# eloialonso/diamond

Hardware: AMD Instinct MI355X
Metric: imagined frames/sec (64x64, 3 denoise steps, batch 256) (higher is better)
Workload: dtype f32 via split-f16 MFMA (world-model convs (3x3 stride 1 / 2, 1x1): fp32 operands split into 2 x fp16 pieces, 3 x v_mfma_f32_*_f16 per product, fp32 accumulate (fp32-class, 22-bit operands); attention core, linears: exact fp32 v_mfma_f32_16x16x4_f32; actor-critic encoder forward, dgrad and weight-gra

## Files before the change

diamond_amd/csrc/dmd_conv.hip:

```cpp
#include <stdlib.h>

#include "dmd_common.h"

#define DMD_CIN_MAX 256

template <int WN_, bool CFGB_, int TAPS_, int STRIDE_, bool SPLIT_ = false>
struct ConvGeom {
  static constexpr bool SPLIT = SPLIT_;
  static constexpr int WN = WN_;
  static constexpr int WM = 4 / WN_;
  static constexpr int MB = 8 / WM;
  static constexpr bool CFGB = CFGB_;
  static constexpr int SUB = CFGB_ ? 2 : 1;
  static constexpr int TH = 8;
  static constexpr int TW = CFGB_ ? 8 : 16;
  static constexpr int TAPS = TAPS_;
  static constexpr int S = STRIDE_;
  static constexpr int PAD = TAPS_ == 9 ? 1 : 0;
  static constexpr int PH = (TH - 1) * STRIDE_ + 1 + 2 * PAD;
  static constexpr int PW = (TW - 1) * STRIDE_ + 1 + 2 * PAD;
  static constexpr int NPP = SUB * PH * PW;
  static constexpr int ITEMS = (NPP * 4 + 255) / 256;
  static constexpr int NBUF = STRIDE_ == 2 ? 1 : 2;
  static constexpr int MIN_WAVES = (WN_ == 4 && CFGB_ && TAPS_ == 9 && STRIDE_ == 1) ? 1 : 2;
  static constexpr bool GENG = false;
};

template <int WN_, bool CFGB_, int TAPS_, int STRIDE_, bool SPLIT_ = false>
struct ConvGeomGN : ConvGeom<WN_, CFGB_, TAPS_, STRIDE_, SPLIT_> {
  static constexpr bool GENG = true;
};

template <class G>
__device__ __forceinline__ void conv_norm_entry(const dmd_norm& nm, int n, int c, int C, int hv, int wv, float* m, float* a, float* ad) {
  if (G::GENG) {
    const int gs = dmd_gn_group_size(C);
    norm_entry_gs(nm, n, c, C, gs, (double)gs * hv * wv, m, a, ad);
  } else {
    norm_entry(nm, n, c, C, (double)DMD_GN_GROUP * hv * wv, m, a, ad);
  }
}

typedef _Float16 h4 __attribute__((ext_vector_type(4)));

__device__ __forceinline__ f32x4 split_h4l4(f32x4 v) {
  h4 hh, ll;
#pragma unroll
  for (int e = 0; e < 4; ++e) {
    hh[e] = (_Float16)v[e];
    ll[e] = (_Float16)(v[e] - (float)hh[e]);
  }
  const uint2 a = __builtin_bit_cast(uint2, hh), b = __builtin_bit_cast(uint2, ll);
  return __builtin_bit_cast(f32x4, (uint4){a.x, a.y, b.x, b.y});
}

struct TileInfo {
  int n, y0, x0;
  bool valid;
};

template <class G>
__device__ __forceinline__ TileInfo decode_subtile(const dmd_conv_params& p, int tile, int s) {
  const int tiles_x = p.W / G::TW, tiles_y = p.H / G::TH;
  const int per_img = tiles_x * tiles_y;
  const int gs = tile * G::SUB + s;
  TileInfo t;
  t.valid = gs < p.N * per_img;
  const int g2 = t.valid ? gs : 0;
  t.n = g2 / per_img;
  const int r = g2 - t.n * per_img;
  const int ty = r / tiles_x;
  t.y0 = ty * G::TH;
  t.x0 = (r - ty * tiles_x) * G::TW;
  return t;
}

template <int SUB>
__device__ __forceinline__ TileInfo pick_tile(const TileInfo* ti, int s) {
  return (SUB == 2 && s) ? ti[SUB - 1] : ti[0];
}

template <class G>
__global__ __launch_bounds__(256, G::MIN_WAVES) void conv_mfma_kernel(const dmd_conv_params p) {
  __shared__ f32x4 patch[G::NBUF][G::NPP * 4];
  __shared__ float tab_mean[G::SUB][DMD_CIN_MAX];
  __shared__ float tab_a[G::SUB][DMD_CIN_MAX];
  __shared__ float tab_add[G::SUB][DMD_CIN_MAX];
  __shared__ float rtab[G::SUB][3][64];
  __shared__ double red[G::SUB][4][2];

  const int tid = threadIdx.x;
  const int lane = tid & 63;
  const int wave = tid >> 6;
  const int wn = wave % G::WN;
  const int wm = wave / G::WN;
  const int j = lane & 15;
  const int kg = lane >> 4;
  const int tile = blockIdx.x;
  const int cout_group0 = blockIdx.y * (16 * G::WN);

  TileInfo ti[G::SUB];
#pragma unroll
  for (int s = 0; s < G::SUB; ++s) ti[s] = decode_subtile<G>(p, tile, s);

  const int up = p.upsample;
  const int Hin = p.H * G::S, Win = p.W * G::S;
  const int Hs = Hin >> up, Ws = Win >> up;
  const int Hvo = p.valid_h ? p.valid_h : p.H, Wvo = p.valid_w ? p.valid_w : p.W;
  const int Hvi = Hvo * G::S, Wvi = Wvo * G::S;
  const int Hvs = Hvi >> up, Wvs = Wvi >> up;
  const int C0 = p.src[0].C;
  const int C1 = p.nsrc > 1 ? p.src[1].C : 0;
  const int nch0 = C0 >> 4;
  const int nchunks = (C0 + C1) >> 4;

  for (int c = tid; c < C0 + C1; c += 256) {
    const int si = c < C0 ? 0 : 1;
    const dmd_conv_src& sc = p.src[si];
    const int cl = si ? c - C0 : c;
#pragma unroll
    for (int s = 0; s < G::SUB; ++s) {
      float m = 0.f, a = 1.f, ad = 0.f;
      if (sc.prologue != DMD_PROLOGUE_NONE && ti[s].valid)
        conv_norm_entry<G>(sc.norm, ti[s].n, cl, sc.C, Hvs, Wvs, &m, &a, &ad);
      tab_mean[s][c] = m;
      tab_a[s][c] = a;
      tab_add[s][c] = ad;
    }
  }
  if (p.residual_norm.stats) {
    for (int c = tid; c < 16 * G::WN; c += 256) {
#pragma unroll
      for (int s = 0; s < G::SUB; ++s) {
        float m = 0.f, a = 1.f, ad = 0.f;
        const int cc = cout_group0 + c;
        if (ti[s].valid && cc < p.Cout)
          conv_norm_entry<G>(p.residual_norm, ti[s].n, cc, p.Cout, Hvo, Wvo, &m, &a, &ad);
        rtab[s][0][c] = m;
        rtab[s][1][c] = a;
        rtab[s][2][c] = ad;
      }
    }
  }

  int goff[G::ITEMS];
  int loff[G::ITEMS];
  int isub[G::ITEMS];
  const int q = tid & 3;
#pragma unroll
  for (int it = 0; it < G::ITEMS; ++it) {
    const int id = it * 256 + tid;
    const int pp = id >> 2;
    const bool ok = pp < G::NPP;
    const int s = G::SUB == 1 ? 0 : (pp >= G::PH * G::PW ? 1 : 0);
    const TileInfo t = pick_tile<G::SUB>(ti, s);
    const int rem = pp - s * (G::PH * G::PW);
    const int py = rem / G::PW;
    const int px = rem - py * G::PW;
    const int iy = t.y0 * G::S - G::PAD + py;
    const int ix = t.x0 * G::S - G::PAD + px;
    const bool inb = ok && t.valid && iy >= 0 && iy < Hvi && ix >= 0 && ix < Wvi;
    goff[it] = inb ? ((t.n * Hs + (iy >> up)) * Ws + (ix >> up)) : -1;
    loff[it] = ok ? pp * 4 + ((q + 2 * (pp >> 2)) & 3) : -1;
    isub[it] = s;
  }

  int pixbase[G::MB];
#pragma unroll
  for (int mb = 0; mb < G::MB; ++mb) {
    const int gmb = wm * G::MB + mb;
    int s, y, x;
    if (G::CFGB) {
      s = gmb >> 2;
      y = (gmb & 3) * 2 + (j >> 3);
      x = j & 7;
    } else {
      s = 0;
      y = gmb;
      x = j;
    }
    pixbase[mb] = s * (G::PH * G::PW) + (y * G::S) * G::PW + x * G::S;
  }

  f32x4 acc[G::MB];
#pragma unroll
  for (int mb = 0; mb < G::MB; ++mb) acc[mb] = (f32x4){0.f, 0.f, 0.f, 0.f};

  const size_t wstep = (size_t)p.CoutPad * 16;
  const float* wlane = p.w + (size_t)(cout_group0 + 16 * wn + j) * 16 + 4 * kg;

  f32x4 stage[G::ITEMS];
  auto load_chunk = [&](int ck) {
    const int si = ck < nch0 ? 0 : 1;
    const dmd_conv_src& sc = p.src[si];
    const int c0 = (si ? ck - nch0 : ck) * 16 + 4 * q;
#pragma unroll
    for (int it = 0; it < G::ITEMS; ++it) {
      stage[it] = (f32x4){0.f, 0.f, 0.f, 0.f};
      if (goff[it] >= 0) stage[it] = *(const f32x4*)(sc.x + (size_t)goff[it] * sc.C + c0);
    }
  };
  const bool fast_math = p.precision != DMD_PRECISION_F32;
  auto store_chunk = [&](int ck, int buf) {
    const int si = ck < nch0 ? 0 : 1;
    const int prologue = p.src[si].prologue;
    const int cc = ck * 16 + 4 * q;
#pragma unroll
    for (int it = 0; it < G::ITEMS; ++it) {
      f32x4 v = stage[it];
      if (prologue != DMD_PROLOGUE_NONE && goff[it] >= 0) {
        const int s = isub[it];
#pragma unroll
        for (int e = 0; e < 4; ++e) {
          float t = (v[e] - tab_mean[s][cc + e]) * tab_a[s][cc + e] + tab_add[s][cc + e];
          if (prologue == DMD_PROLOGUE_NORM_SILU) t = fast_math ? dmd_silu_fast(t) : dmd_silu(t);
          v[e] = t;
        }
      }
      if (G::SPLIT) v = split_h4l4(v);
      if (loff[it] >= 0) patch[buf][loff[it]] = v;
    }
  };

  f32x4 wreg[G::TAPS];
  auto load_weights = [&](int ck, f32x4 (&dst)[G::TAPS]) {
#pragma unroll
    for (int tap = 0; tap < G::TAPS; ++tap) dst[tap] = *(const f32x4*)(wlane + (size_t)(ck * G::TAPS + tap) * wstep);
  };

  __syncthreads();
  load_chunk(0);
  load_weights(0, wreg);
  store_chunk(0, 0);
  __syncthreads();

  for (int ck = 0; ck < nchunks; ++ck) {
    const int buf = G::NBUF == 2 ? (ck & 1) : 0;
    const bool more = ck + 1 < nchunks;
    if (more) load_chunk(ck + 1);
#pragma unroll
    for (int tap = 0; tap < G::TAPS; ++tap) {
      const int dy = G::TAPS == 9 ? tap / 3 : 0;
      const int dx = G::TAPS == 9 ? tap % 3 : 0;
      const f32x4 wf = wreg[tap];
      if (G::SPLIT) {
        const uint4 wb = __builtin_bit_cast(uint4, split_h4l4(wf));
        const h4 wh = __builtin_bit_cast(h4, (uint2){wb.x, wb.y}), wl = __builtin_bit_cast(h4, (uint2){wb.z, wb.w});
#pragma unroll
        for (int mb = 0; mb < G::MB; ++mb) {
          const int pix = pixbase[mb] + dy * G::PW + dx;
          const uint4 xb = __builtin_bit_cast(uint4, patch[buf][pix * 4 + ((kg + 2 * (pix >> 2)) & 3)]);
          const h4 xh = __builtin_bit_cast(h4, (uint2){xb.x, xb.y}), xl = __builtin_bit_cast(h4, (uint2){xb.z, xb.w});
          acc[mb] = __builtin_amdgcn_mfma_f32_16x16x16f16(wh, xl, acc[mb], 0, 0, 0);
          acc[mb] = __builtin_amdgcn_mfma_f32_16x16x16f16(wl, xh, acc[mb], 0, 0, 0);
          acc[mb] = __builtin_amdgcn_mfma_f32_16x16x16f16(wh, xh, acc[mb], 0, 0, 0);
        }
        __builtin_amdgcn_sched_barrier(0);
        continue;
      }
#pragma unroll
      for (int mb = 0; mb < G::MB; ++mb) {
        const int pix = pixbase[mb] + dy * G::PW + dx;
        const f32x4 xf = patch[buf][pix * 4 + ((kg + 2 * (pix >> 2)) & 3)];
        acc[mb] = __builtin_amdgcn_mfma_f32_16x16x4f32(wf[0], xf[0], acc[mb], 0, 0, 0);
        acc[mb] = __builtin_amdgcn_mfma_f32_16x16x4f32(wf[1], xf[1], acc[mb], 0, 0, 0);
        acc[mb] = __builtin_amdgcn_mfma_f32_16x16x4f32(wf[2], xf[2], acc[mb], 0, 0, 0);
        acc[mb] = __builtin_amdgcn_mfma_f32_16x16x4f32(wf[3], xf[3], acc[mb], 0, 0, 0);
      }
    }
    if (more) load_weights(ck + 1, wreg);
    if (G::NBUF == 1) __syncthreads();
    if (more) store_chunk(ck + 1, G::NBUF == 2 ? (buf ^ 1) : 0);
    __syncthreads();
  }

  const int cl = 16 * wn + 4 * kg;
  const int cq = cout_group0 + cl;
  f32x4 bias = (f32x4){0.f, 0.f, 0.f, 0.f};
  if (p.bias) bias = *(const f32x4*)(p.bias + cq);
  double ssum[G::SUB], ssq[G::SUB];
#pragma unroll
  for (int s = 0; s < G::SUB; ++s) ssum[s] = ssq[s] = 0.0;

#pragma unroll
  for (int mb = 0; mb < G::MB; ++mb) {
    const int gmb = wm * G::MB + mb;
    int s, y, x;
    if (G::CFGB) {
      s = gmb >> 2;
      y = (gmb & 3) * 2 + (j >> 3);
      x = j & 7;
    } else {
      s = 0;
      y = gmb;
      x = j;
    }
    const TileInfo t = pick_tile<G::SUB>(ti, s);
    if (!t.valid) continue;
    const int oy = t.y0 + y, ox = t.x0 + x;
    const size_t pixel = ((size_t)t.n * p.H + oy) * p.W + ox;
    f32x4 v = acc[mb] + bias;
    if (p.residual) {
      if (cq + 3 < p.Cout && (p.Cout & 3) == 0) {
        f32x4 r = *(const f32x4*)(p.residual + pixel * p.Cout + cq);
        if (p.residual_norm.stats) {
#pragma unroll
          for (int e = 0; e < 4; ++e) r[e] = (r[e] - rtab[s][0][cl + e]) * rtab[s][1][cl + e] + rtab[s][2][cl + e];
        }
        v += r;
      } else {
        for (int e = 0; e < 4; ++e)
          if (cq + e < p.Cout) {
            float r = p.residual[pixel * p.Cout + cq + e];
            if (p.residual_norm.stats) r = (r - rtab[s][0][cl + e]) * rtab[s][1][cl + e] + rtab[s][2][cl + e];
            v[e] += r;
          }
      }
    }
    if (p.out_nchw) {
      for (int e = 0; e < 4; ++e)
        if (cq + e < p.Cout) p.out[(((size_t)t.n * p.Cout + cq + e) * p.H + oy) * p.W + ox] = v[e];
    } else if (cq + 3 < p.Cout && (p.Cout & 3) == 0) {
      *(f32x4*)(p.out + pixel * p.Cout + cq) = v;
    } else {
      for (int e = 0; e < 4; ++e)
        if (cq + e < p.Cout) p.out[pixel * p.Cout + cq + e] = v[e];
    }
    constexpr bool kBoth = G::CFGB && G::WM == 1;
    const bool counted = oy < Hvo && ox < Wvo;
#pragma unroll
    for (int e = 0; e < 4; ++e) {
      const double d = counted ? (double)v[e] : 0.0;
      if (kBoth && mb >= G::MB / 2) {
        ssum[G::SUB - 1] += d;
        ssq[G::SUB - 1] += d * d;
      } else {
        ssum[0] += d;
        ssq[0] += d * d;
      }
    }
  }

  if (p.out_stats) {
    constexpr bool kBoth = G::CFGB && G::WM == 1;
    const int swave = G::CFGB ? ((wm * G::MB) >> 2) : 0;
#pragma unroll
    for (int s = 0; s < G::SUB; ++s) {
      const double a = dmd_wave_sum(ssum[kBoth ? s : 0]);
      const double b = dmd_wave_sum(ssq[kBoth ? s : 0]);
      if (lane == 0) {
        const bool mine = kBoth || s == swave;
        red[s][wave][0] = mine ? a : 0.0;
        red[s][wave][1] = mine ? b : 0.0;
      }
    }
    __syncthreads();
    constexpr int NG = G::WN / 2 > 0 ? G::WN / 2 : 1;
    if (tid < G::SUB * NG) {
      const int s = tid / NG, g = tid % NG;
      const TileInfo t = pick_tile<G::SUB>(ti, s);
      if (t.valid) {
        double a = 0.0, b = 0.0;
        for (int w = 0; w < 4; ++w) {
          if (((w % G::WN) >> 1) == g) {
            a += red[s][w][0];
            b += red[s][w][1];
          }
        }
        const int tiles_x = p.W / G::TW, tiles_y = p.H / G::TH;
        const int T = tiles_x * tiles_y;
        const int tt = (t.y0 / G::TH) * tiles_x + t.x0 / G::TW;
        const int Gt = p.Cout / DMD_GN_GROUP;
        const int gg = cout_group0 / DMD_GN_GROUP + g;
        double* o = p.out_stats + ((size_t)(t.n * Gt + gg) * T + tt) * 2;
        o[0] = a;
        o[1] = b;
      }
    }
  }
}

__global__ void conv_naive_kernel(const dmd_conv_params p, int stat_tw) {
  const size_t total = (size_t)p.N * p.H * p.W * p.Cout;
  const size_t idx = (size_t)blockIdx.x * blockDim.x + threadIdx.x;
  if (idx >= total) return;
  const int co = idx % p.Cout;
  const size_t pixel = idx / p.Cout;
  const int ox = pixel % p.W;
  const int oy = (pixel / p.W) % p.H;
  const int n = pixel / ((size_t)p.W * p.H);
  const int S = p.stride, up = p.upsample, pad = p.taps == 9 ? 1 : 0, k = p.taps == 9 ? 3 : 1;
  const int Hin = p.H * S, Win = p.W * S, Hs = Hin >> up, Ws = Win >> up;
  const int Hvo = p.valid_h ? p.valid_h : p.H, Wvo = p.valid_w ? p.valid_w : p.W;
  const int Hvi = Hvo * S, Wvi = Wvo * S, Hvs = Hvi >> up, Wvs = Wvi >> up;
  float acc = 0.f;
  int cbase = 0;
  for (int si = 0; si < p.nsrc; ++si) {
    const dmd_conv_src& sc = p.src[si];
    for (int c = 0; c < sc.C; ++c) {
      float m = 0.f, a = 1.f, ad = 0.f;
      if (sc.prologue != DMD_PROLOGUE_NONE) norm_entry(sc.norm, n, c, sc.C, (double)DMD_GN_GROUP * Hvs * Wvs, &m, &a, &ad);
      const int cc = cbase + c;
      for (int dy = 0; dy < k; ++dy)
        for (int dx = 0; dx < k; ++dx) {
          const int iy = oy * S - pad + dy, ix = ox * S - pad + dx;
          if (iy < 0 || iy >= Hvi || ix < 0 || ix >= Wvi) continue;
          float v = sc.x[(((size_t)n * Hs + (iy >> up)) * Ws + (ix >> up)) * sc.C + c];
          if (sc.prologue != DMD_PROLOGUE_NONE) {
            v = (v - m) * a + ad;
            if (sc.prologue == DMD_PROLOGUE_NORM_SILU) v = dmd_silu(v);
          }
          const float w = p.w[(((size_t)(cc >> 4) * p.taps + dy * k + dx) * p.CoutPad + co) * 16 + (cc & 15)];
          acc = fmaf(w, v, acc);
        }
    }
    cbase += sc.C;
  }
  if (p.bias) acc += p.bias[co];
  if (p.residual) {
    float r = p.residual[pixel * p.Cout + co];
    if (p.residual_norm.stats) {
      float m, a, ad;
      norm_entry(p.residual_norm, n, co, p.Cout, (double)DMD_GN_GROUP * Hvo * Wvo, &m, &a, &ad);
      r = (r - m) * a + ad;
    }
    acc += r;
  }
  if (p.out_nchw)
    p.out[(((size_t)n * p.Cout + co) * p.H + oy) * p.W + ox] = acc;
  else
    p.out[idx] = acc;
}

__global__ void conv_naive_stats_kernel(const float* out, double* stats, int N, int H, int W, int C, int TW, int Hv, int Wv) {
  const int tiles_x = W / TW, tiles_y = H / 8, T = tiles_x * tiles_y, G = C / DMD_GN_GROUP;
  const int idx = blockIdx.x * blockDim.x + threadIdx.x;
  if (idx >= N * G * T) return;
  const int t = idx % T, g = (idx / T) % G, n = idx / (T * G);
  const int y0 = (t / tiles_x) * 8, x0 = (t % tiles_x) * TW;
  double s = 0.0, ss = 0.0;
  for (int y = 0; y < 8; ++y)
    for (int x = 0; x < TW; ++x)
      for (int c = 0; c < DMD_GN_GROUP; ++c) {
        if (y0 + y >= Hv || x0 + x >= Wv) continue;
        const double v = out[(((size_t)n * H + y0 + y) * W + x0 + x) * C + g * DMD_GN_GROUP + c];
        s += v;
        ss += v * v;
      }
  stats[(size_t)idx * 2] = s;
  stats[(size_t)idx * 2 + 1] = ss;
}

__global__ void pack_weight_kernel(const float* oihw, float* packed, int Cout, int Cin, int k, int CoutPad, int CinPad) {
  const int taps = k * k;
  const size_t total = (size_t)(CinPad / 16) * taps * CoutPad * 16;
  const size_t idx = (size_t)blockIdx.x * blockDim.x + threadIdx.x;
  if (idx >= total) return;
  const int ci = idx % 16;
  const int co = (idx / 16) % CoutPad;
  const int tap = (idx / (16 * (size_t)CoutPad)) % taps;
  const int chunk = idx / (16 * (size_t)CoutPad * taps);
  const int c = chunk * 16 + ci;
  float v = 0.f;
  if (co < Cout && c < Cin) v = oihw[((size_t)co * Cin + c) * taps + tap];
  packed[idx] = v;
}

extern "C" int dmd_conv2d_proj_eligible(const dmd_conv_params* p);
static int validate_conv(const dmd_conv_params* p) {
  DMD_CHECK_ARG(p != nullptr, "conv: null params");
  DMD_CHECK_ARG(p->N > 0 && p->H > 0 && p->W > 0, "conv: bad N/H/W %d %d %d", p->N, p->H, p->W);
  DMD_CHECK_ARG(p->H % 8 == 0 && p->W % 8 == 0, "conv: H, W must be multiples of 8 (got %d x %d)", p->H, p->W);
  DMD_CHECK_ARG(p->taps == 9 || p->taps == 1, "conv: taps must be 9 or 1");
  DMD_CHECK_ARG(p->stride == 1 || (p->stride == 2 && p->taps == 9), "conv: bad stride");
  DMD_CHECK_ARG(!(p->upsample && p->stride != 1), "conv: upsample with stride");
  DMD_CHECK_ARG(p->nsrc == 1 || p->nsrc == 2, "conv: nsrc");
  int cin = 0;
  for (int i = 0; i < p->nsrc; ++i) {
    DMD_CHECK_ARG(p->src[i].x && p->src[i].C > 0 && p->src[i].C % 16 == 0, "conv: src %d channels %d", i, p->src[i].C);
    if (p->src[i].prologue != DMD_PROLOGUE_NONE) {
      DMD_CHECK_ARG(p->src[i].norm.stats && p->src[i].norm.stat_tiles > 0, "conv: src %d prologue without stats", i);
      DMD_CHECK_ARG(dmd_gn_width_ok(p->src[i].C), "conv: normalised source of %d channels (C %% 32 == 0, or C <= 256 in groups of "
                    "C / max(1, C / 32) channels, a multiple of 4)", p->src[i].C);
    }
    cin += p->src[i].C;
  }
  DMD_CHECK_ARG(cin <= DMD_CIN_MAX, "conv: Cin %d > %d", cin, DMD_CIN_MAX);
  DMD_CHECK_ARG(p->Cout > 0 && p->CoutPad >= p->Cout && p->CoutPad % 16 == 0, "conv: Cout/CoutPad");
  DMD_CHECK_ARG(p->w && p->out, "conv: null weight/out");
  if (p->out_stats) DMD_CHECK_ARG(p->Cout % DMD_GN_GROUP == 0 && p->CoutPad == p->Cout, "conv: out_stats needs Cout %% 32 == 0");
  if (p->residual_norm.stats) DMD_CHECK_ARG(p->residual && dmd_gn_width_ok(p->Cout), "conv: residual_norm");
  if (p->upsample) DMD_CHECK_ARG(p->H % 2 == 0 && p->W % 2 == 0, "conv: upsample needs even output");
  DMD_CHECK_ARG(p->valid_h >= 0 && p->valid_h <= p->H && p->valid_w >= 0 && p->valid_w <= p->W && (p->valid_h == 0) == (p->valid_w == 0),
                "conv: valid extent %d x %d outside the %d x %d buffer", p->valid_h, p->valid_w, p->H, p->W);
  if (p->upsample) DMD_CHECK_ARG(p->valid_h % 2 == 0 && p->valid_w % 2 == 0, "conv: upsample needs an even valid extent");
  if (p->proj_nsrc)
    DMD_CHECK_ARG(dmd_conv2d_proj_eligible(p), "conv: fused skip projection on parameters dmd_conv2d_proj_eligible() rejects "
                  "(needs F16X2 3x3 stride 1, Cout 64, H, W %% 16 == 0, two 64-channel sources, no residual)");
  return 0;
}

static bool conv_geng(const dmd_conv_params& p) {
  for (int i = 0; i < p.nsrc; ++i)
    if (p.src[i].prologue != DMD_PROLOGUE_NONE && p.src[i].C % DMD_GN_GROUP != 0) return true;
  return p.residual_norm.stats && p.Cout % DMD_GN_GROUP != 0;
}

static int conv_mfma_split(const dmd_conv_params& p) { return (p.precision & 0xff) == DMD_PRECISION_F16X2; }

template <int WN, bool CFGB, int TAPS, int STRIDE>
static void launch_conv(const dmd_conv_params& p, int groups, hipStream_t st) {
  using G = ConvGeom<WN, CFGB, TAPS, STRIDE>;
  const int tiles = (p.H / G::TH) * (p.W / G::TW) * p.N;
  dim3 grid((tiles + G::SUB - 1) / G::SUB, groups);
  if (conv_geng(p)) {
    if (conv_mfma_split(p))
      hipLaunchKernelGGL((conv_mfma_kernel<ConvGeomGN<WN, CFGB, TAPS, STRIDE, true>>), grid, dim3(256), 0, st, p);
    else
      hipLaunchKernelGGL((conv_mfma_kernel<ConvGeomGN<WN, CFGB, TAPS, STRIDE>>), grid, dim3(256), 0, st, p);
  } else if (conv_mfma_split(p))
    hipLaunchKernelGGL((conv_mfma_kernel<ConvGeom<WN, CFGB, TAPS, STRIDE, true>>), grid, dim3(256), 0, st, p);
  else
    hipLaunchKernelGGL((conv_mfma_kernel<G>), grid, dim3(256), 0, st, p);
}

template <int TAPS, int STRIDE>
static void dispatch_wn(const dmd_conv_params& p, hipStream_t st) {
  const bool cfgb = (p.W % 16) != 0;
  if (p.CoutPad % 64 == 0) {
    cfgb ? launch_conv<4, true, TAPS, STRIDE>(p, p.CoutPad / 64, st) : launch_conv<4, false, TAPS, STRIDE>(p, p.CoutPad / 64, st);
  } else if (p.CoutPad % 32 == 0) {
    cfgb ? launch_conv<2, true, TAPS, STRIDE>(p, p.CoutPad / 32, st) : launch_conv<2, false, TAPS, STRIDE>(p, p.CoutPad / 32, st);
  } else {
    cfgb ? launch_conv<1, true, TAPS, STRIDE>(p, p.CoutPad / 16, st) : launch_conv<1, false, TAPS, STRIDE>(p, p.CoutPad / 16, st);
  }
}

extern "C" int dmd_conv_stat_tiles(int H, int W) { return (H / 8) * (W / ((W % 16) ? 8 : 16)); }

int dmd_launch_conv_f16ws(const dmd_conv_params& p, hipStream_t st);
int dmd_launch_conv1x1_stream(const dmd_conv_params& p, hipStream_t st);
extern "C" int dmd_conv1x1_stream_eligible(const dmd_conv_params* p);

extern "C" int dmd_conv2d(const dmd_conv_params* p, dmd_stream_t stream) {
  if (int e = validate_conv(p)) return e;
  hipStream_t st = (hipStream_t)stream;
  if (dmd_conv1x1_stream_eligible(p)) {
    dmd_launch_conv1x1_stream(*p, st);
  } else if (dmd_conv2d_f16x2_eligible(p)) {
    if (int e = dmd_launch_conv_f16ws(*p, st)) return e;
  } else if (p->taps == 1)
    dispatch_wn<1, 1>(*p, st);
  else if (p->stride == 2)
    dispatch_wn<9, 2>(*p, st);
  else
    dispatch_wn<9, 1>(*p, st);
  DMD_LAUNCH_CHECK();
  return 0;
}

extern "C" int dmd_conv2d_kernel_name(const dmd_conv_params* p, char* buf, int buf_len) {
  if (int e = validate_conv(p)) return e;
  DMD_CHECK_ARG(buf && buf_len > 0, "kernel_name: buffer");
  const bool b8 = p->W % 16 != 0;
  if (dmd_conv1x1_stream_eligible(p)) {
    int cin = 0;
    for (int i = 0; i < p->nsrc; ++i) cin += p->src[i].C;
    snprintf(buf, buf_len, "conv1x1_stream_kernel<%d, %d, %s>", cin / 16, cin == 128 ? 2 : 4,
             (p->precision & 0xff) == DMD_PRECISION_F16X2 ? "true" : "false");
  } else if (p->proj_nsrc) {
    snprintf(buf, buf_len, "conv_f16ws_kernel<WsGeomProj>");
  } else if (dmd_conv2d_f16x2_eligible(p)) {
    snprintf(buf, buf_len, "conv_f16ws_kernel<WsGeom<%s, %d, %d>>", b8 ? "true" : "false", p->CoutPad == 64 ? 2 : 1, p->taps);
  } else {
    const int wn = p->CoutPad % 64 == 0 ? 4 : (p->CoutPad % 32 == 0 ? 2 : 1);
    snprintf(buf, buf_len, "conv_mfma_kernel<%s<%d, %s, %d, %d, %s>>", conv_geng(*p) ? "ConvGeomGN" : "ConvGeom", wn, b8 ? "true" : "false", p->taps, p->stride,
             conv_mfma_split(*p) ? "true" : "false");
  }
  return 0;
}

extern "C" int dmd_conv2d_naive(const dmd_conv_params* p, dmd_stream_t stream) {
  if (int e = validate_conv(p)) return e;
  DMD_CHECK_ARG(!p->proj_nsrc, "naive conv: no fused skip projection (run the projection as its own launch)");
  DMD_CHECK_ARG(!conv_geng(*p), "naive conv: normalisation in groups of 32 channels only");
  hipStream_t st = (hipStream_t)stream;
  const size_t total = (size_t)p->N * p->H * p->W * p->Cout;
  dmd_conv_params q = *p;
  float* tmp_out = p->out;
  hipLaunchKernelGGL(conv_naive_kernel, dim3((unsigned)((total + 255) / 256)), dim3(256), 0, st, q, 0);
  if (p->out_stats) {
    DMD_CHECK_ARG(!p->out_nchw, "naive conv: stats need NHWC output");
    const int TW = (p->W % 16) ? 8 : 16;
    const int n = p->N * (p->Cout / DMD_GN_GROUP) * dmd_conv_stat_tiles(p->H, p->W);
    hipLaunchKernelGGL(conv_naive_stats_kernel, dim3((n + 63) / 64), dim3(64), 0, st, tmp_out, p->out_stats, p->N, p->H,
                       p->W, p->Cout, TW, p->valid_h ? p->valid_h : p->H, p->valid_w ? p->valid_w : p->W);
  }
  DMD_LAUNCH_CHECK();
  return 0;
}

extern "C" int dmd_pack_conv_weight(const float* oihw, float* packed, int Cout, int Cin, int k, int CoutPad, int CinPad,
                                    dmd_stream_t stream) {
  DMD_CHECK_ARG(oihw && packed, "pack: null");
  DMD_CHECK_ARG((k == 1 || k == 3) && CoutPad >= Cout && CoutPad % 16 == 0 && CinPad >= Cin && CinPad % 16 == 0,
                "pack: bad sizes");
  const size_t total = (size_t)(CinPad / 16) * k * k * CoutPad * 16;
  hipLaunchKernelGGL(pack_weight_kernel, dim3((unsigned)((total + 255) / 256)), dim3(256), 0, (hipStream_t)stream, oihw,
                     packed, Cout, Cin, k, CoutPad, CinPad);
  DMD_LAUNCH_CHECK();
  return 0;
}
```

Baseline: 13010.

## Add persistent streaming 3x3 conv kernel for Cout=32 layers with prefetch pipeline

Adds a persistent kernel for 3x3 stride-1 convolutions with 16 or 32 input and 32 output channels. It keeps the split-f16 weights resident in LDS, loops over 16x16 pixel tile pairs, and prefetches the next tile's input into registers while the current tile runs on 32x32x16 MFMA. The group-norm and SiLU prologue, residual add and output statistics are fused in, and the path is routed only for shapes flagged as measured faster. The aim is to hide global-load latency and cut per-tile weight reloads and launch overhead, at the cost of high register pressure and shape-specific heuristics.

After: 12830. -1.4%, worse.

```diff
diff --git a/diamond_amd/csrc/dmd_conv.hip b/diamond_amd/csrc/dmd_conv.hip
--- a/diamond_amd/csrc/dmd_conv.hip
+++ b/diamond_amd/csrc/dmd_conv.hip
@@ -541,12 +541,19 @@
 int dmd_launch_conv_f16ws(const dmd_conv_params& p, hipStream_t st);
 int dmd_launch_conv1x1_stream(const dmd_conv_params& p, hipStream_t st);
 extern "C" int dmd_conv1x1_stream_eligible(const dmd_conv_params* p);
+int dmd_conv_stream32_route(const dmd_conv_params& p) __attribute__((weak));
+int dmd_launch_conv_stream32(const dmd_conv_params& p, hipStream_t st) __attribute__((weak));
+static int conv_stream32(const dmd_conv_params& p) {
+  return (dmd_conv_stream32_route && dmd_launch_conv_stream32) ? dmd_conv_stream32_route(p) : 0;
+}
 
 extern "C" int dmd_conv2d(const dmd_conv_params* p, dmd_stream_t stream) {
   if (int e = validate_conv(p)) return e;
   hipStream_t st = (hipStream_t)stream;
   if (dmd_conv1x1_stream_eligible(p)) {
     dmd_launch_conv1x1_stream(*p, st);
+  } else if (conv_stream32(*p)) {
+    if (int e = dmd_launch_conv_stream32(*p, st)) return e;
   } else if (dmd_conv2d_f16x2_eligible(p)) {
     if (int e = dmd_launch_conv_f16ws(*p, st)) return e;
   } else if (p->taps == 1)
@@ -570,6 +577,8 @@
              (p->precision & 0xff) == DMD_PRECISION_F16X2 ? "true" : "false");
   } else if (p->proj_nsrc) {
     snprintf(buf, buf_len, "conv_f16ws_kernel<WsGeomProj>");
+  } else if (const int nch = conv_stream32(*p)) {
+    snprintf(buf, buf_len, "conv_f16ws_stream32_kernel<%d>", nch);
   } else if (dmd_conv2d_f16x2_eligible(p)) {
     snprintf(buf, buf_len, "conv_f16ws_kernel<WsGeom<%s, %d, %d>>", b8 ? "true" : "false", p->CoutPad == 64 ? 2 : 1, p->taps);
   } else {
diff --git a/diamond_amd/csrc/dmd_conv_f16s32.hip b/diamond_amd/csrc/dmd_conv_f16s32.hip
--- /dev/null
+++ b/diamond_amd/csrc/dmd_conv_f16s32.hip
@@ -0,0 +1,411 @@
+#include <type_traits>
+
+#include "dmd_common.h"
+
+namespace {
+
+typedef _Float16 h8 __attribute__((ext_vector_type(8)));
+typedef _Float16 h2 __attribute__((ext_vector_type(2)));
+typedef float f32x16 __attribute__((ext_vector_type(16)));
+typedef unsigned int u32x4 __attribute__((ext_vector_type(4)));
+
+constexpr int S32_PW = 18, S32_PPS = S32_PW * S32_PW;
+constexpr int S32_NPP = 2 * S32_PPS;
+constexpr int S32_ITEMS = (S32_NPP * 4 + 255) / 256;
+constexpr int S32_W_BYTES = 9 * 2 * 2 * 32 * 16;
+constexpr int S32_PATCH_BYTES = S32_NPP * 64;
+constexpr int S32_RES_BATCH = 2;
+constexpr int S32_TAB_FLOATS = 2 * 32;
+constexpr int s32_smem_bytes(int nch) { return nch * S32_W_BYTES + S32_PATCH_BYTES + 4 * S32_TAB_FLOATS * 4 + 32 * 4; }
+
+template <int I, int N, class F>
+__device__ __forceinline__ void s32_for(F&& f) {
+  if constexpr (I < N) {
+    f(std::integral_constant<int, I>{});
+    s32_for<I + 1, N>(f);
+  }
+}
+
+__device__ __forceinline__ unsigned s32_low_pair(float x0, float x1, unsigned h01) {
+  unsigned l01;
+  asm("v_fma_mixlo_f16 %0, %1, 1.0, -%3 op_sel:[0,0,0] op_sel_hi:[0,0,1]\n\t"
+      "v_fma_mixhi_f16 %0, %2, 1.0, -%3 op_sel:[0,0,1] op_sel_hi:[0,0,1]"
+      : "=&v"(l01)
+      : "v"(x0), "v"(x1), "v"(h01));
+  return l01;
+}
+
+#define S32_OPAQUE(t) asm volatile("" : "+v"(t))
+
+__device__ __forceinline__ void s32_barrier() { asm volatile("s_waitcnt lgkmcnt(0)\n\ts_barrier" ::: "memory"); }
+
+typedef const __attribute__((address_space(1))) char* s32_gptr;
+__device__ __forceinline__ s32_gptr s32_uniform_ptr(const char* p) {
+  const unsigned long long v = (unsigned long long)p;
+  const unsigned lo = __builtin_amdgcn_readfirstlane((unsigned)v), hi = __builtin_amdgcn_readfirstlane((unsigned)(v >> 32));
+  return (s32_gptr)(((unsigned long long)hi << 32) | lo);
+}
+
+template <int CTRL, int ROW_MASK>
+__device__ __forceinline__ double s32_dpp_add(double x) {
+  const unsigned long long u = __builtin_bit_cast(unsigned long long, x);
+  const unsigned lo = (unsigned)__builtin_amdgcn_update_dpp(0, (int)(unsigned)u, CTRL, ROW_MASK, 0xf, false);
+  const unsigned hi = (unsigned)__builtin_amdgcn_update_dpp(0, (int)(unsigned)(u >> 32), CTRL, ROW_MASK, 0xf, false);
+  return x + __builtin_bit_cast(double, (unsigned long long)lo | ((unsigned long long)hi << 32));
+}
+__device__ __forceinline__ double s32_wave_sum_lane63(double x) {
+  x = s32_dpp_add<0xB1, 0xf>(x);
+  x = s32_dpp_add<0x4E, 0xf>(x);
+  x = s32_dpp_add<0x141, 0xf>(x);
+  x = s32_dpp_add<0x140, 0xf>(x);
+  x = s32_dpp_add<0x142, 0xa>(x);
+  x = s32_dpp_add<0x143, 0xc>(x);
+  return x;
+}
+
+struct S32Tile {
+  int n, y0, x0;
+  bool valid;
+};
+__device__ __forceinline__ S32Tile s32_subtile(const dmd_conv_params& p, int tile, int s) {
+  const int tx = p.W / 16, per_img = tx * (p.H / 16);
+  const int gs = tile * 2 + s;
+  S32Tile t;
+  t.valid = gs < p.N * per_img;
+  const int g2 = t.valid ? gs : 0;
+  t.n = g2 / per_img;
+  const int r = g2 - t.n * per_img;
+  const int ty = r / tx;
+  t.y0 = ty * 16;
+  t.x0 = (r - ty * tx) * 16;
+  return t;
+}
+
+}
+
+template <int NCH>
+__global__ __launch_bounds__(256, 2) void conv_f16ws_stream32_kernel(const dmd_conv_params p, int ntiles) {
+  DMD_DYNAMIC_LDS(unsigned char, smem_raw);
+  unsigned char* const patch = smem_raw;
+  float* const tab_a = (float*)(patch + S32_PATCH_BYTES);
+  float* const tab_b = tab_a + S32_TAB_FLOATS;
+  float* const tab_c = tab_b + S32_TAB_FLOATS;
+  float* const tab_d = tab_c + S32_TAB_FLOATS;
+  float* const bias_lds = tab_d + S32_TAB_FLOATS;
+  unsigned char* const w_lds = (unsigned char*)(bias_lds + 32);
+  static_assert(2 * s32_smem_bytes(NCH) <= 160 * 1024, "two workgroups per CU");
+
+  const int tid = (int)threadIdx.x;
+  const int lane = tid & 63, wave = __builtin_amdgcn_readfirstlane(tid >> 6);
+  const int q = tid & 3;
+  const int n31 = lane & 31, g = lane >> 5;
+  const int C = 16 * NCH;
+  const int nwg = (int)gridDim.x, wg = (int)blockIdx.x;
+  const int base_n = ntiles / nwg, extra = ntiles - base_n * nwg;
+  const int tile0 = wg * base_n + min(wg, extra);
+  const int nmy = base_n + (wg < extra ? 1 : 0);
+  if (nmy <= 0) return;
+  const int rot = (int)((blockIdx.x * 7u) % (unsigned)nmy);
+  auto tile_of = [&](int k) { return tile0 + (k + rot >= nmy ? k + rot - nmy : k + rot); };
+
+  {
+    const u32x4* wg = (const u32x4*)p.w_f16;
+    for (int u = tid; u < NCH * S32_W_BYTES / 16; u += 256) ((u32x4*)w_lds)[u] = wg[u];
+    if (tid < 32) bias_lds[tid] = p.bias ? p.bias[tid] : 0.f;
+  }
+
+  const int pp0 = tid >> 2;
+  int tab_n0 = -1, tab_n1 = -1;
+  auto write_tables = [&](int tile) {
+    const S32Tile t0 = s32_subtile(p, tile, 0), t1 = s32_subtile(p, tile, 1);
+    const int n0 = t0.valid ? t0.n : -2, n1 = t1.valid ? t1.n : -2;
+    if (n0 == tab_n0 && n1 == tab_n1) return;
+    tab_n0 = n0;
+    tab_n1 = n1;
+    if (tid < 2 * C) {
+      const int s = tid / C, c = tid - s * C;
+      const S32Tile t = s ? t1 : t0;
+      const dmd_conv_src& sc = p.src[0];
+      float m = 0.f, a = 1.f, ad = 0.f;
+      if (sc.prologue != DMD_PROLOGUE_NONE && t.valid) norm_entry(sc.norm, t.n, c, sc.C, (double)DMD_GN_GROUP * p.H * p.W, &m, &a, &ad);
+      const float bb = ad - m * a;
+      const bool silu = sc.prologue == DMD_PROLOGUE_NORM_SILU;
+      const int ti = s * 32 + c;
+      tab_a[ti] = a;
+      tab_b[ti] = bb;
+      tab_c[ti] = silu ? -1.4426950408889634f * a : 0.f;
+      tab_d[ti] = silu ? -1.4426950408889634f * bb : -126.f;
+    }
+  };
+
+  f32x4 st[NCH][S32_ITEMS];
+  int goff[S32_ITEMS];
+  unsigned zm_req = 0;
+  unsigned zm_cur = 0;
+  auto setup_request = [&](int tile) {
+    const S32Tile t0 = s32_subtile(p, tile, 0), t1 = s32_subtile(p, tile, 1);
+    unsigned gz = 0;
+    int pq = pp0;
+    S32_OPAQUE(pq);
+#pragma unroll
+    for (int it = 0; it < S32_ITEMS; ++it) {
+      const int pp = it * 64 + pq;
+      const int s = pp >= S32_PPS ? 1 : 0;
+      const int rem = pp - s * S32_PPS;
+      const int py = rem / S32_PW, px = rem - py * S32_PW;
+      const S32Tile t = s ? t1 : t0;
+      const int iy = t.y0 - 1 + py, ix = t.x0 - 1 + px;
+      const bool inb = (pp < S32_NPP) & t.valid & (iy >= 0) & (iy < p.H) & (ix >= 0) & (ix < p.W);
+      goff[it] = inb ? (t.n * p.H + iy) * p.W + ix : 0;
+      gz |= (inb ? 0u : 1u) << it;
+    }
+    zm_req = gz;
+  };
+  auto request = [&](auto ckc) {
+    constexpr int ck = decltype(ckc)::value;
+    const s32_gptr base = s32_uniform_ptr((const char*)p.src[0].x + ck * 64);
+#pragma unroll
+    for (int it = 0; it < S32_ITEMS; ++it) {
+      const unsigned voff = __umul24((unsigned)goff[it], (unsigned)(C * 4)) + 16u * q;
+      st[ck][it] = *(const __attribute__((address_space(1))) f32x4*)(base + voff);
+    }
+  };
+  auto stage = [&](auto ckc) {
+    constexpr int ck = decltype(ckc)::value;
+    const int cc = ck * 16 + 4 * q;
+    uint2* pb = (uint2*)patch;
+    f32x4 ta[2], tb[2], tc[2], td[2];
+    auto load_tab = [&](int s) {
+      ta[s] = *(const f32x4*)(tab_a + s * 32 + cc);
+      tb[s] = *(const f32x4*)(tab_b + s * 32 + cc);
+      tc[s] = *(const f32x4*)(tab_c + s * 32 + cc);
+      td[s] = *(const f32x4*)(tab_d + s * 32 + cc);
+    };
+    load_tab(0);
+    int pq = pp0;
+    S32_OPAQUE(pq);
+    s32_for<0, S32_ITEMS>([&](auto ic) {
+      constexpr int it = decltype(ic)::value;
+      const int pp = it * 64 + pq;
+      if constexpr (it == 5) {
+        __builtin_amdgcn_sched_barrier(0);
+        load_tab(1);
+      }
+      if constexpr (it == 6) __builtin_amdgcn_sched_barrier(0);
+      const bool s1 = it > 5 || (it == 5 && pp >= S32_PPS);
+      float t[4], u[4];
+#pragma unroll
+      for (int el = 0; el < 4; ++el) {
+        const float a = s1 ? ta[1][el] : ta[0][el], b = s1 ? tb[1][el] : tb[0][el];
+        const float c = s1 ? tc[1][el] : tc[0][el], d = s1 ? td[1][el] : td[0][el];
+        t[el] = __builtin_fmaf(st[ck][it][el], a, b);
+        u[el] = __builtin_fmaf(st[ck][it][el], c, d);
+      }
+#pragma unroll
+      for (int el = 0; el < 4; ++el) u[el] = __builtin_amdgcn_exp2f(u[el]);
+#pragma unroll
+      for (int el = 0; el < 4; ++el) u[el] = 1.0f + u[el];
+#pragma unroll
+      for (int el = 0; el < 4; ++el) u[el] = __builtin_amdgcn_rcpf(u[el]);
+      const bool zero = (zm_cur >> it) & 1;
+#pragma unroll
+      for (int el = 0; el < 4; ++el) {
+        const float y = t[el] * u[el];
+        u[el] = zero ? 0.f : y;
+      }
+      const unsigned h01 = __builtin_bit_cast(unsigned, (h2){(_Float16)u[0], (_Float16)u[1]});
+      const unsigned h23 = __builtin_bit_cast(unsigned, (h2){(_Float16)u[2], (_Float16)u[3]});
+      const unsigned l01 = s32_low_pair(u[0], u[1], h01);
+      const unsigned l23 = s32_low_pair(u[2], u[3], h23);
+      if (it + 1 < S32_ITEMS || pp < S32_NPP) {
+        const int s = pp >= S32_PPS ? 1 : 0;
+        const int rem = pp - s * S32_PPS;
+        const int px = rem - (rem / S32_PW) * S32_PW;
+        const int lo = (pp * 4 + (((q >> 1) + (px >> 1)) & 3)) * 2 + (q & 1);
+        pb[lo] = (uint2){h01, h23};
+        pb[lo ^ 4] = (uint2){l01, l23};
+      }
+    });
+  };
+
+  int ph_addr[3];
+  {
+    const int col = n31 & 15;
+    const int pixbase = (wave >> 1) * S32_PPS + ((wave & 1) * 8 + (n31 >> 4)) * S32_PW + col;
+#pragma unroll
+    for (int dx = 0; dx < 3; ++dx) ph_addr[dx] = (pixbase * 4 + ((g + ((col + dx) >> 1)) & 3)) * 16;
+  }
+  const int w_addr = (g * 32 + n31) * 16;
+
+  f32x16 acc[4];
+  auto mfma_chunk = [&](auto ckc) {
+    constexpr int ck = decltype(ckc)::value;
+    const unsigned char* wl = w_lds + ck * S32_W_BYTES + w_addr;
+    s32_for<0, 9>([&](auto tc_) {
+      constexpr int tap = decltype(tc_)::value;
+      constexpr int dy = tap / 3, dx = tap % 3;
+      const h8 ah = *(const h8*)(wl + (tap * 2 + 0) * 2 * 32 * 16);
+      const h8 al = *(const h8*)(wl + (tap * 2 + 1) * 2 * 32 * 16);
+      h8 bh[4], bl[4];
+#pragma unroll
+      for (int blk = 0; blk < 4; ++blk) {
+        const int off = ((dy + 2 * blk) * S32_PW + dx) * 64;
+        bh[blk] = *(const h8*)(patch + ph_addr[dx] + off);
+        bl[blk] = *(const h8*)(patch + (ph_addr[dx] ^ 32) + off);
+      }
+#pragma unroll
+      for (int blk = 0; blk < 4; ++blk) acc[blk] = __builtin_amdgcn_mfma_f32_32x32x16_f16(ah, bh[blk], acc[blk], 0, 0, 0);
+#pragma unroll
+      for (int blk = 0; blk < 4; ++blk) acc[blk] = __builtin_amdgcn_mfma_f32_32x32x16_f16(ah, bl[blk], acc[blk], 0, 0, 0);
+#pragma unroll
+      for (int blk = 0; blk < 4; ++blk) acc[blk] = __builtin_amdgcn_mfma_f32_32x32x16_f16(al, bh[blk], acc[blk], 0, 0, 0);
+      __builtin_amdgcn_sched_barrier(0);
+    });
+  };
+
+  auto epilogue = [&](int tile) {
+    const S32Tile t = s32_subtile(p, tile, wave >> 1);
+    if (!t.valid) return;
+    const int oy = t.y0 + (wave & 1) * 8 + (n31 >> 4), ox = t.x0 + (n31 & 15);
+    const int po0 = ((t.n * p.H + oy) * p.W + ox) * 8 + g;
+    double ssum = 0, ssq = 0;
+    f32x4 r[4][4];
+#pragma unroll
+    for (int blk = 0; blk < 4; ++blk) {
+      const size_t po = (size_t)(po0 + blk * 2 * p.W * 8);
+      float* op = p.out + po * 4;
+      if (blk % S32_RES_BATCH == 0) {
+        if (p.residual) {
+#pragma unroll
+          for (int b2 = blk; b2 < blk + S32_RES_BATCH; ++b2)
+#pragma unroll
+            for (int qd = 0; qd < 4; ++qd) r[b2][qd] = *(const f32x4*)(p.residual + (size_t)(po0 + b2 * 2 * p.W * 8) * 4 + 8 * qd);
+        } else {
+#pragma unroll
+          for (int b2 = blk; b2 < blk + S32_RES_BATCH; ++b2)
+#pragma unroll
+            for (int qd = 0; qd < 4; ++qd) r[b2][qd] = (f32x4){0.f, 0.f, 0.f, 0.f};
+        }
+      }
+      f32x4 v[4];
+#pragma unroll
+      for (int qd = 0; qd < 4; ++qd) {
+        v[qd] = (f32x4){acc[blk][4 * qd], acc[blk][4 * qd + 1], acc[blk][4 * qd + 2], acc[blk][4 * qd + 3]};
+#pragma unroll
+        for (int e = 0; e < 4; ++e) v[qd][e] += r[blk][qd][e];
+      }
+      float fs = 0.f, fq = 0.f;
+#pragma unroll
+      for (int qd = 0; qd < 4; ++qd) {
+        *(f32x4*)(op + 8 * qd) = v[qd];
+        fs += (v[qd][0] + v[qd][1]) + (v[qd][2] + v[qd][3]);
+        fq = __builtin_fmaf(v[qd][0], v[qd][0], fq);
+        fq = __builtin_fmaf(v[qd][1], v[qd][1], fq);
+        fq = __builtin_fmaf(v[qd][2], v[qd][2], fq);
+        fq = __builtin_fmaf(v[qd][3], v[qd][3], fq);
+      }
+      ssum += (double)fs;
+      ssq += (double)fq;
+    }
+    if (p.out_stats) {
+      const double a = s32_wave_sum_lane63(ssum);
+      const double b = s32_wave_sum_lane63(ssq);
+      if (lane == 63) {
+        const int tx16 = p.W / 16, T = tx16 * (p.H / 8);
+        const int tt = (t.y0 / 8 + (wave & 1)) * tx16 + t.x0 / 16;
+        double* o = p.out_stats + ((size_t)t.n * T + tt) * 2;
+        o[0] = a;
+        o[1] = b;
+      }
+    }
+  };
+
+  auto advance = [&](int k) {
+    zm_cur = zm_req;
+    stage(std::integral_constant<int, 0>{});
+    if (k + 1 < nmy) {
+      setup_request(tile_of(k + 1));
+      request(std::integral_constant<int, 0>{});
+    }
+  };
+  write_tables(tile_of(0));
+  setup_request(tile_of(0));
+  s32_for<0, NCH>([&](auto ckc) { request(ckc); });
+  s32_barrier();
+  advance(0);
+  for (int k = 0; k < nmy; ++k) {
+    const bool more = k + 1 < nmy;
+    s32_for<0, NCH>([&](auto ckc) {
+      constexpr int ck = decltype(ckc)::value;
+      if constexpr (ck > 0) {
+        stage(ckc);
+        if (more) request(ckc);
+      }
+      s32_barrier();
+      if constexpr (ck == 0) {
+        f32x4 bq[4];
+#pragma unroll
+        for (int qd = 0; qd < 4; ++qd) bq[qd] = *(const f32x4*)(bias_lds + 8 * qd + 4 * g);
+#pragma unroll
+        for (int blk = 0; blk < 4; ++blk)
+#pragma unroll
+          for (int r = 0; r < 16; ++r) acc[blk][r] = bq[r >> 2][r & 3];
+      }
+      mfma_chunk(ckc);
+      if (ck == NCH - 1 && more) write_tables(tile_of(k + 1));
+      s32_barrier();
+    });
+    if (more) advance(k + 1);
+    epilogue(tile_of(k));
+  }
+}
+
+template <int NCH>
+static int launch_stream32(const dmd_conv_params& p, int ntiles, int max_wg, hipStream_t st) {
+  static bool attr_set[DMD_MAX_DEVICES] = {};
+  static int ncus[DMD_MAX_DEVICES] = {};
+  int dev = 0;
+  if (hipGetDevice(&dev) != hipSuccess || dev < 0 || dev >= DMD_MAX_DEVICES) dev = 0;
+  constexpr int SMEM = s32_smem_bytes(NCH);
+  if (!attr_set[dev]) {
+    hipError_t e = hipFuncSetAttribute(reinterpret_cast<const void*>(&conv_f16ws_stream32_kernel<NCH>),
+                                       hipFuncAttributeMaxDynamicSharedMemorySize, SMEM);
+    DMD_CHECK_ARG(e == hipSuccess, "conv_f16ws_stream32: hipFuncSetAttribute(%d bytes): %s", SMEM, hipGetErrorString(e));
+    int n = 0;
+    if (hipDeviceGetAttribute(&n, hipDeviceAttributeMultiprocessorCount, dev) != hipSuccess || n <= 0) n = 256;
+    ncus[dev] = n;
+    attr_set[dev] = true;
+  }
+  int nwg = 2 * ncus[dev];
+  if (max_wg > 0 && max_wg < nwg) nwg = max_wg;
+  if (ntiles < nwg) nwg = ntiles;
+  hipLaunchKernelGGL((conv_f16ws_stream32_kernel<NCH>), dim3(nwg), dim3(256), SMEM, st, p, ntiles);
+  return 0;
+}
+
+static DmdEnvInt s32_switch{"DIAMOND_CONV32_STREAM", 1};
+static DmdEnvInt s32_max_wg{"DIAMOND_CONV32_STREAM_MAX_WG", 0};
+static bool s32_measured_faster(const dmd_conv_params& p) {
+  if ((long long)p.N * p.H * p.W < 512ll * 512) return false;
+  const int C = p.src[0].C;
+  if (p.H == 64 && p.W == 64) return C == 16;
+  if (p.H == 32 && p.W == 32) return C == 32 && (p.src[0].prologue != DMD_PROLOGUE_NONE || !p.residual);
+  return false;
+}
+
+int dmd_conv_stream32_route(const dmd_conv_params& p) {
+  const int sw = s32_switch.get();
+  if (sw == 0 || !dmd_conv2d_f16x2_eligible(&p)) return 0;
+  if (p.taps != 9 || p.upsample || p.proj_nsrc || p.Cout != 32 || p.CoutPad != 32 || p.out_nchw) return 0;
+  if (p.nsrc != 1 || (p.src[0].C != 16 && p.src[0].C != 32)) return 0;
+  if (p.H % 16 != 0 || p.W % 16 != 0 || p.valid_h || p.valid_w) return 0;
+  const long long pixels = (long long)p.N * p.H * p.W;
+  if (pixels * 32 * 4 >= (1ll << 32)) return 0;
+  if (sw == 1 && !s32_measured_faster(p)) return 0;
+  return p.src[0].C / 16;
+}
+
+int dmd_launch_conv_stream32(const dmd_conv_params& p, hipStream_t st) {
+  const int ntiles = (p.N * (p.H / 16) * (p.W / 16) + 1) / 2;
+  return p.src[0].C == 16 ? launch_stream32<1>(p, ntiles, s32_max_wg.get(), st) : launch_stream32<2>(p, ntiles, s32_max_wg.get(), st);
+}
```
